# armando-palacio/opticomlib

Measured on AMD Instinct MI355X. Metric: SSFM sample*steps/sec, 2^20-sample dual-pol fiber, higher is better.
Workload: dtype c64

## Files before the change

opticomlib_amd/csrc/ssfm_host.hip:

```cpp
#include <hip/hip_runtime.h>

#include <algorithm>
#include <memory>
#include <cmath>
#include <cstdarg>
#include <cstddef>
#include <cstdio>
#include <cstdlib>
#include <chrono>
#include <cstring>
#include <atomic>
#include <condition_variable>
#include <functional>
#include <mutex>
#include <new>
#include <string>
#include <thread>
#include <type_traits>
#include <vector>

#include "ssfm_amd.h"
#include "ssfm_common.hpp"
#include "ssfm_kernels.hpp"
#include "ssfm_launch.hpp"
#include "ssfm_medium.hpp"
#include "ssfm_owned.hpp"
#include "ssfm_schedule.hpp"
#include "ssfm_split.hpp"

using namespace ssfm;

namespace {

constexpr int kLog2Min = 8, kLog2Max = 24;
constexpr int kLog2MaxDirect = 22;
template <typename T> constexpr int cols_per_tile() { return sizeof(T) == 8 ? 8 : 16; }
constexpr int kMaxTables = 4;

constexpr int freq_rows(int n2, int e) { return (n2 / e) >= 64 ? 1 : ((64 * e / n2) > 16 ? 16 : (64 * e / n2)); }

template <typename T, int MODE, int N1, int E>
hipError_t launch_time_n1(dim3 grid, hipStream_t s, const TimeArgs<T>& a) {
    constexpr int C = cols_per_tile<T>();
    constexpr bool U16 = u16_layout<T>(N1, C, E);
    if constexpr (!U16 && MODE > TM_END && MODE != TM_MID_A && MODE != TM_MID_L) return hipErrorInvalidValue;
    else if constexpr (U16 && MODE == TM_MID_L) return hipErrorInvalidValue;
    else if constexpr (MODE == TM_MID_A && N1 != 128 && N1 != 256) return hipErrorInvalidValue;
    else {
    constexpr size_t lds = col_pass_lds<T>(N1, C, E);
    if constexpr (MODE == TM_BEGIN || MODE == TM_MID || MODE == TM_END) {
        if (a.scal != nullptr)
            return launch_kernel<k_time<T, N1, C, E, MODE, U16, true>, lds>(grid, dim3(N1 * C / E), s, SSFM_TIME_KERNEL_ARGS(a));
    }
    return launch_kernel<k_time<T, N1, C, E, MODE, U16>, lds>(grid, dim3(N1 * C / E), s, SSFM_TIME_KERNEL_ARGS(a));
    }
}
template <typename T, int MODE, int E>
hipError_t launch_time_e(int N1, int batch, hipStream_t s, const TimeArgs<T>& a) {
    const dim3 grid((unsigned)(a.N2 / cols_per_tile<T>()) * batch);
    switch (N1) {
        case 16:  return launch_time_n1<T, MODE, 16, E>(grid, s, a);
        case 32:  return launch_time_n1<T, MODE, 32, E>(grid, s, a);
        case 64:  return launch_time_n1<T, MODE, 64, E>(grid, s, a);
        case 128: return launch_time_n1<T, MODE, 128, E>(grid, s, a);
        case 256: return launch_time_n1<T, MODE, 256, E>(grid, s, a);
        case 512: if constexpr (E == 16) return launch_time_n1<T, MODE, 512, E>(grid, s, a); else break;
    }
    return hipErrorInvalidValue;
}
template <typename T, int MODE>
hipError_t launch_time(int N1, int batch, hipStream_t s, TimeArgs<T> a, int E) {
    a.rows = batch;
    return E == 8 ? launch_time_e<T, MODE, 8>(N1, batch, s, a) : launch_time_e<T, MODE, 16>(N1, batch, s, a);
}

template <typename T, int MODE, int N2, int E, bool U16>
hipError_t launch_freq_u(int nrows, hipStream_t s, const FreqArgs<T>& a) {
    constexpr int ROWS = freq_rows(N2, E);
    constexpr size_t lds = row_pass_lds<T>(N2, E, ROWS);
    if constexpr (MODE == FM_FWD_ONLY || MODE == FM_INV_ONLY)
        return launch_kernel<k_freq_half<T, N2, ROWS, E, MODE, U16>, lds>(dim3(nrows / ROWS), dim3(ROWS * N2 / E), s, SSFM_FREQ_KERNEL_ARGS(a));
    else
        return launch_kernel<k_freq<T, N2, ROWS, E, MODE, U16>, lds>(dim3(nrows / ROWS), dim3(ROWS * N2 / E), s, SSFM_FREQ_KERNEL_ARGS(a));
}
template <typename T, int MODE, int N2, int E>
hipError_t launch_freq_n2(int nrows, hipStream_t s, const FreqArgs<T>& a) {
    if constexpr (sizeof(T) == 4)
        if (a.u16) return launch_freq_u<T, MODE, N2, E, true>(nrows, s, a);
    if constexpr ((MODE == FM_PHASE && sizeof(T) == 4) || MODE == FM_FLY_IM) return hipErrorInvalidValue;
    else return launch_freq_u<T, MODE, N2, E, false>(nrows, s, a);
}
template <typename T, int MODE, int E>
hipError_t launch_freq_e(int N2, int nrows, hipStream_t s, const FreqArgs<T>& a) {
    if constexpr (MODE == FM_INV_ONLY) {
        switch (N2) {
            case 4096: return launch_freq_n2<T, MODE, 4096, E>(nrows, s, a);
            case 8192: if constexpr (E == 16) return launch_freq_n2<T, MODE, 8192, E>(nrows, s, a); else break;
        }
        return hipErrorInvalidValue;
    } else
    switch (N2) {
        case 16:   return launch_freq_n2<T, MODE, 16, E>(nrows, s, a);
        case 32:   return launch_freq_n2<T, MODE, 32, E>(nrows, s, a);
        case 64:   return launch_freq_n2<T, MODE, 64, E>(nrows, s, a);
        case 128:  return launch_freq_n2<T, MODE, 128, E>(nrows, s, a);
        case 256:  return launch_freq_n2<T, MODE, 256, E>(nrows, s, a);
        case 512:  return launch_freq_n2<T, MODE, 512, E>(nrows, s, a);
        case 1024: return launch_freq_n2<T, MODE, 1024, E>(nrows, s, a);
        case 2048: return launch_freq_n2<T, MODE, 2048, E>(nrows, s, a);
        case 4096: return launch_freq_n2<T, MODE, 4096, E>(nrows, s, a);
        case 8192: if constexpr (E == 16) return launch_freq_n2<T, MODE, 8192, E>(nrows, s, a); else break;
    }
    return hipErrorInvalidValue;
}
template <typename T, int MODE>
hipError_t launch_freq(int N2, int nrows, hipStream_t s, FreqArgs<T> a, int E) {
    a.rows = nrows / a.N1;
    return E == 8 ? launch_freq_e<T, MODE, 8>(N2, nrows, s, a) : launch_freq_e<T, MODE, 16>(N2, nrows, s, a);
}

template <int MODE, int N1, int E>
hipError_t launch_time_h_n1(dim3 grid, hipStream_t s, const TimeArgs<double>& a) {
    constexpr int C = cols_per_tile<double>();
    return launch_kernel<k_time_h<double, N1, C, E, MODE>, col_pass_lds<double>(N1, C, E)>(grid, dim3(N1 * C / E), s, SSFM_TIME_KERNEL_ARGS(a));
}
constexpr bool line_half_shape(int N1, int N2, int E, int Ef) { return ((N1 == 256 && E == 8) || (N1 == 512 && E == 16)) && Ef == 16 && N2 >= 1024 && N2 <= 8192; }
template <int MODE>
hipError_t launch_time_h(int N1, int batch, hipStream_t s, TimeArgs<double> a, int E) {
    a.rows = batch;
    const dim3 grid((unsigned)(a.N2 / cols_per_tile<double>()) * batch);
    if (N1 == 256 && E == 8) return launch_time_h_n1<MODE, 256, 8>(grid, s, a);
    if (N1 == 512 && E == 16) return launch_time_h_n1<MODE, 512, 16>(grid, s, a);
    return hipErrorInvalidValue;
}
template <int N2>
hipError_t launch_freq_h_n2(int nrows, hipStream_t s, const FreqArgs<double>& a, const int* done) {
    constexpr int E = 16, ROWS = freq_rows(N2, E);
    constexpr auto kernel = &k_freq_h<double, N2, ROWS, E, FM_TABLE>;
    constexpr size_t lds = row_pass_lds<double>(N2, E, ROWS);
    const dim3 grid(nrows / ROWS), block(ROWS * N2 / E);
#if SSFM_TRACE
    return launch_kernel<kernel, lds>(grid, block, s, a.F, a.tab, a.tw2, a.st, a.h, a.amp, a.inv_n, a.step, a.N1, a.rows, a.u16, done, a.trace, a.trace_slot);
#else
    return launch_kernel<kernel, lds>(grid, block, s, a.F, a.tab, a.tw2, a.st, a.h, a.amp, a.inv_n, a.step, a.N1, a.rows, a.u16, done);
#endif
}
inline hipError_t launch_freq_h(int N2, int nrows, hipStream_t s, FreqArgs<double> a, const int* done = nullptr) {
    a.rows = nrows / a.N1;
    switch (N2) {
        case 1024: return launch_freq_h_n2<1024>(nrows, s, a, done);
        case 2048: return launch_freq_h_n2<2048>(nrows, s, a, done);
        case 4096: return launch_freq_h_n2<4096>(nrows, s, a, done);
        case 8192: return launch_freq_h_n2<8192>(nrows, s, a, done);
    }
    return hipErrorInvalidValue;
}

template <typename T, int MODE, int R>
hipError_t launch_split_mid_r(hipStream_t s, const SplitArgs<T>& a) {
    constexpr int V = split_positions<T, R>();
    const long long units = (long long)a.N1 * a.N2 / V;
    hipLaunchKernelGGL((k_split_mid<T, R, MODE>), dim3((unsigned)((units + 255) / 256)), dim3(256), 0, s, a);
    return hipGetLastError();
}
template <typename T, int MODE>
hipError_t launch_split_mid(int R, hipStream_t s, const SplitArgs<T>& a) {
    switch (R) {
        case 2:  return launch_split_mid_r<T, MODE, 2>(s, a);
        case 4:  return launch_split_mid_r<T, MODE, 4>(s, a);
        case 8:  return launch_split_mid_r<T, MODE, 8>(s, a);
        case 16: return launch_split_mid_r<T, MODE, 16>(s, a);
    }
    return hipErrorInvalidValue;
}
template <typename T, bool TO_SUB>
hipError_t launch_split_shuffle(int R, hipStream_t s, cx<T>* sub, cx<T>* nat, long long M, int rows) {
    const dim3 grid((unsigned)((M * rows + 255) / 256));
    switch (R) {
        case 2:  hipLaunchKernelGGL((k_split_shuffle<T, 2, TO_SUB>), grid, dim3(256), 0, s, sub, nat, M, rows); break;
        case 4:  hipLaunchKernelGGL((k_split_shuffle<T, 4, TO_SUB>), grid, dim3(256), 0, s, sub, nat, M, rows); break;
        case 8:  hipLaunchKernelGGL((k_split_shuffle<T, 8, TO_SUB>), grid, dim3(256), 0, s, sub, nat, M, rows); break;
        case 16: hipLaunchKernelGGL((k_split_shuffle<T, 16, TO_SUB>), grid, dim3(256), 0, s, sub, nat, M, rows); break;
        default: return hipErrorInvalidValue;
    }
    return hipGetLastError();
}

constexpr int kSmallE16Min = 4096;
template <typename T> constexpr int small_points(int n) { return sizeof(T) == 4 && n >= kSmallE16Min ? 16 : 8; }
template <typename T> constexpr bool small_supported(int n) {
    return n >= 256 && n <= (sizeof(T) == 4 ? 8192 : 4096) && (n & (n - 1)) == 0;
}
static_assert(kSmallTabs == kMaxTables, "k_small takes one table per cached step size");
template <int MAXN, typename F>
hipError_t small_size(int n, F&& f) {
    switch (n) {
        case 256:  return f(std::integral_constant<int, 256>());
        case 512:  return f(std::integral_constant<int, 512>());
        case 1024: return f(std::integral_constant<int, 1024>());
        case 2048: return f(std::integral_constant<int, 2048>());
        case 4096: return f(std::integral_constant<int, 4096>());
        case 8192: if constexpr (MAXN >= 8192) return f(std::integral_constant<int, 8192>()); else break;
    }
    return hipErrorInvalidValue;
}
template <typename T>
hipError_t launch_small(int n, int rows, hipStream_t s, const SmallArgs<T>& a) {
    return small_size<(sizeof(T) == 4 ? 8192 : 4096)>(n, [&](auto size) {
        constexpr int N = decltype(size)::value, E = small_points<T>(N);
        return launch_kernel<k_small<T, N, E>, row_pass_lds<T>(N, E, 1)>(dim3(rows), dim3(N / E), s, a);
    });
}

template <typename T> __device__ __forceinline__ cx<T> cm_chirp_value(long long m, long long n, int conj) {
    const long long r = (m * m) % (2 * n);
    double sn, cs;
    sincospi(-(double)r / (double)n, &sn, &cs);
    return mk<T>((T)cs, (T)(conj ? -sn : sn));
}
template <typename T> __global__ __launch_bounds__(256) void k_cm_kernel_line(cx<T>* __restrict__ F, long long n, long long M, int which) {
    for (long long i = (long long)blockIdx.x * blockDim.x + threadIdx.x; i < M; i += (long long)gridDim.x * blockDim.x) {
        const long long m = i < n ? i : (M - i < n ? M - i : -1);
        F[i] = m < 0 ? mk<T>((T)0, (T)0) : cm_chirp_value<T>(m, n, which == 0);
    }
}
template <typename T> __global__ __launch_bounds__(256) void k_cm_mul_table(const cx<T>* __restrict__ Dt, cx<T>* __restrict__ out, long long n, long long M, T h, T inv) {
    for (long long i = (long long)blockIdx.x * blockDim.x + threadIdx.x; i < M; i += (long long)gridDim.x * blockDim.x) {
        cx<T> d = mk<T>((T)0, (T)0);
        if (i < n) {
            const cx<T> x = Dt[i];
            const T xr = x.x * h, xi = x.y * h;
            const T e = (T)exp((double)xr);
            double sn, cs;
            sincos((double)xi, &sn, &cs);
            d = mk<T>((e * (T)cs) * inv, (e * (T)sn) * inv);
        }
        out[i] = d;
    }
}
__global__ __launch_bounds__(256) void k_cm_narrow(const cx<double>* __restrict__ src, cx<float>* __restrict__ dst, long long M, int conj) {
    for (long long i = (long long)blockIdx.x * blockDim.x + threadIdx.x; i < M; i += (long long)gridDim.x * blockDim.x)
        dst[i] = mk<float>((float)src[i].x, (float)(conj ? -src[i].y : src[i].y));
}
template <typename T> __global__ __launch_bounds__(256) void k_cm_pre(const cx<T>* __restrict__ A, const cx<T>* __restrict__ chirp, cx<T>* __restrict__ F, long long n, long long M, int batch) {
    const long long total = M * batch;
    for (long long i = (long long)blockIdx.x * blockDim.x + threadIdx.x; i < total; i += (long long)gridDim.x * blockDim.x) {
        const long long r = i / M, m = i - r * M;
        F[i] = m < n ? cmul(A[r * n + m], chirp[m]) : mk<T>((T)0, (T)0);
    }
}
template <typename T> __global__ __launch_bounds__(256) void k_cm_post(cx<T>* __restrict__ A, const cx<T>* __restrict__ chirp, const cx<T>* __restrict__ F, long long n, long long M, int batch,
                                                                      const unsigned* __restrict__ error) {
    if (*error != 0u) return;
    const long long total = n * batch;
    for (long long i = (long long)blockIdx.x * blockDim.x + threadIdx.x; i < total; i += (long long)gridDim.x * blockDim.x) {
        const long long r = i / n, m = i - r * n;
        A[i] = cmulc(F[r * M + m], chirp[m]);
    }
}

template <typename T> constexpr int chirp_points(int n) { return small_points<T>(n); }
template <typename T>
hipError_t launch_small_chirp(int n, int rows, hipStream_t s, const SmallChirpArgs<T>& a) {
    return small_size<4096>(n, [&](auto size) {
        constexpr int N = decltype(size)::value, E = chirp_points<T>(N);
        constexpr size_t lds = row_pass_lds<T>(N, E, 1, N);
        static_assert(lds <= 160 * 1024, "k_small_chirp: the line, its twiddles and H must fit the LDS");
        return launch_kernel<k_small_chirp<T, N, E>, lds>(dim3(rows), dim3(N / E), s, a);
    });
}
template <typename T>
hipError_t launch_small_chirp_adapt(int n, int rows, hipStream_t s, const SmallChirpAdaptArgs<T>& a) {
    return small_size<4096>(n, [&](auto size) {
        constexpr int N = decltype(size)::value, E = chirp_points<T>(N);
        constexpr size_t lds = row_pass_lds<T>(N, E, 1, N);
        static_assert(lds + 256 <= 160 * 1024, "k_small_chirp_adapt: the line, its twiddles and H must fit the LDS");
        return launch_kernel<k_small_chirp_adapt<T, N, E>, lds>(dim3(rows), dim3(N / E), s, a);
    });
}

template <typename T> constexpr bool small_adapt_supported(int n, int rows) {
    return small_supported<T>(n) && n <= 4096 && rows >= 1 && rows <= 2 && rows * n / small_points<T>(n) <= 512;
}
template <typename T, int N, int ROWS>
hipError_t launch_small_adapt_nr(hipStream_t s, const SmallAdaptArgs<T>& a) {
    constexpr int E = small_points<T>(N);
    if constexpr (ROWS * N / E <= 512) return launch_kernel<k_small_adapt<T, N, E, ROWS>, row_pass_lds<T>(N, E, ROWS)>(dim3(1), dim3(ROWS * N / E), s, a);
    else return hipErrorInvalidValue;
}
template <typename T>
hipError_t launch_small_adapt(int n, int rows, hipStream_t s, const SmallAdaptArgs<T>& a) {
    return small_size<4096>(n, [&](auto size) {
        constexpr int N = decltype(size)::value;
        return rows == 1 ? launch_small_adapt_nr<T, N, 1>(s, a) : launch_small_adapt_nr<T, N, 2>(s, a);
    });
}

class LaneWorker {
  public:
    ~LaneWorker() { stop(); }
    void start(int device) {
        if (th_.joinable()) return;
        th_ = std::thread([this, device] {
            (void)hipSetDevice(device);
            std::unique_lock<std::mutex> lk(m_);
            for (;;) {
                cv_.wait(lk, [this] { return has_job_ || quit_; });
                if (!has_job_) return;
                std::function<int()> job = std::move(job_);
                has_job_ = false;
                lk.unlock();
                const int rc = job();
                std::string err = rc != SSFM_OK ? std::string(ssfm::g_err) : std::string();
                lk.lock();
                rc_ = rc; err_ = std::move(err); done_ = true;
                cv_.notify_all();
            }
        });
    }
    void submit(std::function<int()> job) {
        std::lock_guard<std::mutex> lk(m_);
        job_ = std::move(job); has_job_ = true; done_ = false;
        cv_.notify_all();
    }
    int wait() {
        std::unique_lock<std::mutex> lk(m_);
        cv_.wait(lk, [this] { return done_; });
        if (rc_ != SSFM_OK) std::snprintf(ssfm::g_err, sizeof(ssfm::g_err), "%s", err_.c_str());
        return rc_;
    }
    void stop() {
        { std::lock_guard<std::mutex> lk(m_); quit_ = true; cv_.notify_all(); }
        if (th_.joinable()) th_.join();
    }
  private:
    std::thread th_;
    std::mutex m_;
    std::condition_variable cv_;
    std::function<int()> job_;
    bool has_job_ = false, done_ = false, quit_ = false;
    int rc_ = SSFM_OK;
    std::string err_;
};

__global__ void k_queue_probe_wait(unsigned* flag, unsigned* seen, long long patience) {
    const long long t0 = wall_clock64();
    unsigned v = 0u;
    while ((v = __hip_atomic_load(flag, __ATOMIC_RELAXED, __HIP_MEMORY_SCOPE_AGENT)) == 0u && wall_clock64() - t0 < patience) __builtin_amdgcn_s_sleep(8);
    *seen = v;
}
__global__ void k_queue_probe_set(unsigned* flag) { __hip_atomic_store(flag, 1u, __ATOMIC_RELAXED, __HIP_MEMORY_SCOPE_AGENT); }
__global__ void k_queue_probe_spin(long long ticks) {
    const long long t0 = wall_clock64();
    while (wall_clock64() - t0 < ticks) __builtin_amdgcn_s_sleep(4);
}
int streams_run_side_by_side(hipStream_t a, hipStream_t b, unsigned* words , hipEvent_t ev) {
    unsigned seen = 0u;
    if (hipMemsetAsync(words, 0, 2 * sizeof(unsigned), a) != hipSuccess) return -1;
    if (hipEventRecord(ev, a) != hipSuccess || hipStreamWaitEvent(b, ev, 0) != hipSuccess) return -1;
    hipLaunchKernelGGL(k_queue_probe_wait, dim3(1), dim3(1), 0, a, words, words + 1, 20000ll);
    hipLaunchKernelGGL(k_queue_probe_set, dim3(1), dim3(1), 0, b, words);
    if (hipGetLastError() != hipSuccess) return -1;
    if (hipMemcpyAsync(&seen, words + 1, sizeof(unsigned), hipMemcpyDeviceToHost, a) != hipSuccess) return -1;
    if (hipStreamSynchronize(a) != hipSuccess || hipStreamSynchronize(b) != hipSuccess) return -1;
    return seen != 0u ? 1 : 0;
}

constexpr float kLaneGoodRatio = 1.6f;
constexpr float kLaneGoodRatioBig = 2.1f;
constexpr float kLaneSlowRatio = 1.8f;
constexpr float kLaneSuspectRatio = 1.3f;
constexpr int kLaneDroppedCooldown = 32;
constexpr int kLaneProbeSteps = 12;
constexpr int kLaneHealsMax = 8;

struct LanePair { int device; hipStream_t main, lane; float score, alone_us, pair_us; };
struct LanePool {
    std::mutex m;
    std::vector<LanePair> free;
    static constexpr size_t kMax = 8;
    bool take(int device, LanePair* out) {
        std::lock_guard<std::mutex> lk(m);
        for (size_t i = free.size(); i-- > 0;)
            if (free[i].device == device) { *out = free[i]; free.erase(free.begin() + (long)i); return true; }
        return false;
    }
    bool give(const LanePair& p) {
        std::lock_guard<std::mutex> lk(m);
        if (free.size() >= kMax) return false;
        free.push_back(p);
        return true;
    }
};
LanePool& lane_pool() { static LanePool* p = new LanePool(); return *p; }
std::atomic<long long> g_lane_ratings{0}, g_lane_pairs_reused{0};

struct PlanBase {
    int precision = 0;
    virtual ~PlanBase() {}
};

constexpr int kMaxLanesConst = 8;
template <typename T> struct PlanT : PlanBase {
    int device = 0;
    int64_t n = 0;
    int batch = 0;
    int N1 = 0, N2 = 0;
    hipStream_t stream = nullptr;
    Event ev0, ev1;
    cx<T>* F = nullptr;
    cx<T>* Y = nullptr;
    T* P = nullptr;
    DeviceBuffer<cx<T>> F_own, Y_own;
    DeviceBuffer<T> P_own;
    DeviceBuffer<cx<T>> twN;
    DeviceBuffer<cx<T>> twA;
    DeviceBuffer<cx<T>> twB;
    DeviceBuffer<cx<T>> tw1;
    DeviceBuffer<cx<T>> tw2;
    DeviceBuffer<cx<T>> dnat;
    DeviceBuffer<cx<T>> dperm;
    DeviceBuffer<cx<T>> dperm_fly;
    DeviceBuffer<T> dimag_fly;
    bool dimag_valid = false;
    DeviceBuffer<cx<T>> tw2_fly;
    DeviceBuffer<cx<T>> scratch;
    DeviceBuffer<cx<T>> xfer_tab[2];
    struct Tab { T h = 0; DeviceBuffer<cx<T>> ptr; bool valid = false; int kind = 0; };
    Tab tabs[kMaxTables];
    bool op_flat_re = false;
    T op_re0 = 0;
    bool phase_tables = true;
    bool force_fly = false;
    int tab_rr = 0;
    bool small = false;
    DeviceBuffer<cx<T>> tw_small;
    DeviceBuffer<cx<T>> tw_chirp;
    DeviceBuffer<cx<T>> dsmall;
    bool medium_ok = true;
    static constexpr size_t kSet = kBarShards + kBarWords + 2;
    DeviceBuffer<unsigned long long> medium_st;
    PinnedBuffer<unsigned> medium_err_host;
    Stream medium_stream2;
    Event medium_ev2;
    bool medium_pending = false;
    bool medium_split_ok = true;
    bool medium_adapt_ok = true;
    static constexpr long long medium_max_samples = 1ll << 17;
    int medium_xcc = -1, medium_xccs = 8;
    std::vector<T> medium_sched;
    double medium_gamma = 0;
    long long medium_patience = 2000000ll;
    bool fused_ok = true;
    DeviceBuffer<cx<T>> fused_backup;
    Tab stabs[kMaxTables];
    int stab_rr = 0;
    DeviceBuffer<T> d_hs;
    std::vector<unsigned char> h_sched;
    DeviceBuffer<AdaptState<T>> st;
    DeviceBuffer<T> zlog;
    bool have_op = false;
    int split_R = 1;
    int64_t n_full = 0;
    int batch_full = 0;
// ... 2368 lines not shown
```

opticomlib_amd/csrc/ssfm_split.hpp:

```cpp
#pragma once
#include "ssfm_kernels.hpp"

namespace ssfm {

constexpr int kSplitLog2M = 20;
constexpr int kSplitMaxR = 16;

enum SplitMode { SM_TABLE = 0, SM_FLY = 1, SM_PHASE = 2 };

template <typename T> struct SplitArgs {
    cx<T>* Y;
    const cx<T>* G;
    const double2* twA;
    const double2* twB;
    const AdaptState<T>* st;
    T h;
    T inv_n;
    T amp;
    int step;
    int N1, N2;
    int rows_outer;
    int Qf;
};
__host__ __device__ __forceinline__ long long split_k2_of_pos(long long pos, int Qf) { return Qf > 0 ? u16_col_of_pos(pos, Qf) : pos; }

template <typename T, int R> __host__ __device__ constexpr int split_positions() { return sizeof(T) == 4 ? 2 : 1; }
template <typename T, int R, int MODE>
__global__ __launch_bounds__(256) void k_split_mid(const SplitArgs<T> a) {
    constexpr int V = split_positions<T, R>();
    typedef T v4_t __attribute__((ext_vector_type(V * 2)));
    const long long M = (long long)a.N1 * a.N2;
    const long long unit = (long long)blockIdx.x * 256 + threadIdx.x;
    if (unit * V >= M) return;
    const long long p0 = unit * V;
    const int k1 = (int)(p0 / a.N2);
    int k2v[V];
#pragma unroll
    for (int v = 0; v < V; ++v) k2v[v] = (int)split_k2_of_pos(p0 % a.N2 + v, a.Qf);
    T h = a.h;
    if (MODE == SM_FLY && a.st != nullptr) {
        const StepState<T> S = a.st->cur[a.step & 1];
        if (S.done || a.st->error != 0u) return;
        h = S.h;
    }
    cx<T> g[R][V];
    if constexpr (MODE == SM_PHASE) {
        typedef unsigned uv_t __attribute__((ext_vector_type(V)));
        const unsigned* Gu = reinterpret_cast<const unsigned*>(a.G);
#pragma unroll
        for (int p = 0; p < R; ++p) {
            const uv_t q = *reinterpret_cast<const uv_t*>(Gu + (long long)p * M + p0);
#pragma unroll
            for (int v = 0; v < V; ++v) g[p][v] = phase32_factor(q[v], a.amp);
        }
    } else {
#pragma unroll
    for (int p = 0; p < R; ++p) {
        const v4_t q = *reinterpret_cast<const v4_t*>(a.G + (long long)p * M + p0);
#pragma unroll
        for (int v = 0; v < V; ++v) g[p][v] = mk<T>(q[2 * v], q[2 * v + 1]);
    }
    }
    if constexpr (MODE == SM_FLY) {
#pragma unroll
        for (int v = 0; v < V; ++v) {
            cx<T> m[R];
            T ph[R];
            bool flat = true;
#pragma unroll
            for (int p = 0; p < R; ++p) { m[p] = g[p][v]; ph[p] = m[p].y * h; flat = flat && (m[p].x == m[0].x); }
            const T e0 = exp_acc<T>(m[0].x * h);
            fly_factors<R>(m, ph, flat, e0, h, a.inv_n);
#pragma unroll
            for (int p = 0; p < R; ++p) g[p][v] = m[p];
        }
    }
    cx<T> w[R][V];
#pragma unroll
    for (int s = 1; s < R; ++s) {
        const double2 A = a.twA[s * a.N1 + k1];
#pragma unroll
        for (int v = 0; v < V; ++v) {
            const double2 B = a.twB[(long long)s * a.N2 + k2v[v]];
            w[s][v] = mk<T>((T)(A.x * B.x - A.y * B.y), (T)(A.x * B.y + A.y * B.x));
        }
    }
    for (int row = 0; row < a.rows_outer; ++row) {
        cx<T>* base = a.Y + (long long)row * R * M + p0;
        cx<T> y[R][V];
#pragma unroll
        for (int s = 0; s < R; ++s) {
            const v4_t q = *reinterpret_cast<const v4_t*>(base + (long long)s * M);
#pragma unroll
            for (int v = 0; v < V; ++v) y[s][v] = mk<T>(q[2 * v], q[2 * v + 1]);
        }
#pragma unroll
        for (int v = 0; v < V; ++v) {
            cx<T> t[R];
            t[0] = y[0][v];
#pragma unroll
            for (int s = 1; s < R; ++s) t[s] = cmul(y[s][v], w[s][v]);
            Dft<R>::template run<-1>(t);
#pragma unroll
            for (int p = 0; p < R; ++p) t[p] = cmul(t[p], g[p][v]);
            Dft<R>::template run<+1>(t);
            y[0][v] = t[0];
#pragma unroll
            for (int s = 1; s < R; ++s) y[s][v] = cmul(t[s], mk<T>(w[s][v].x, -w[s][v].y));
        }
#pragma unroll
        for (int s = 0; s < R; ++s) {
            v4_t q;
#pragma unroll
            for (int v = 0; v < V; ++v) { q[2 * v] = y[s][v].x; q[2 * v + 1] = y[s][v].y; }
            *reinterpret_cast<v4_t*>(base + (long long)s * M) = q;
        }
    }
}

template <typename T, int MODE>
__global__ void k_make_split_table(const cx<T>* __restrict__ src, cx<T>* __restrict__ out, int N1, int N2, int R, T h, T inv_n, int Qf) {
    const long long o = (long long)blockIdx.x * blockDim.x + threadIdx.x;
    const long long M = (long long)N1 * N2;
    if (o >= M * R) return;
    const long long p = o / M, r = o % M;
    const long long k1 = r / N2, k2 = split_k2_of_pos(r % N2, Qf);
    cx<T> d = src[k1 + (long long)N1 * k2 + M * p];
    if (MODE == 1) { d.x *= inv_n; d.y *= inv_n; }
    if (MODE == 2) {
        const T xr = d.x * h, xi = d.y * h;
        const T e = (T)exp((double)xr);
        double s, c;
        sincos((double)xi, &s, &c);
        d.x = (e * (T)c) * inv_n;
        d.y = (e * (T)s) * inv_n;
    }
    out[o] = d;
}
template <typename T>
__global__ void k_make_split_phase_table(const cx<T>* __restrict__ src, unsigned* __restrict__ out, int N1, int N2, int R, T h, int Qf) {
    const long long o = (long long)blockIdx.x * blockDim.x + threadIdx.x;
    const long long M = (long long)N1 * N2;
    if (o >= M * R) return;
    const long long p = o / M, r = o % M;
    const long long k1 = r / N2, k2 = split_k2_of_pos(r % N2, Qf);
    const T xi = src[k1 + (long long)N1 * k2 + M * p].y * h;
    double turns = (double)xi * 0.15915494309189533577;
    turns -= floor(turns);
    out[o] = (unsigned)(unsigned long long)llrint(turns * 4294967296.0);
}
template <typename T>
__global__ void k_make_split_dm_table(cx<T>* __restrict__ out, cx<T>* __restrict__ nat, int N1, int N2, int R, double val, double D, T inv_n, int Qf) {
    const long long o = (long long)blockIdx.x * blockDim.x + threadIdx.x;
    const long long M = (long long)N1 * N2, N = M * R;
    if (o >= N) return;
    const long long p = o / M, r = o % M;
    const long long k = (r / N2) + (long long)N1 * split_k2_of_pos(r % N2, Qf) + M * p;
    const long long ks = k < (N + 1) / 2 ? k : k - N;
    const double w = ((double)ks * val) * 2.0 * 3.141592653589793;
    const double ph = ((w * w) * D) / 2.0;
    double s, c;
    sincos(ph, &s, &c);
    out[o] = mk<T>((T)c * inv_n, (T)s * inv_n);
    if (nat != nullptr) nat[k] = mk<T>((T)c, (T)s);
}
__global__ inline void k_make_split_twiddles(double2* twA, double2* twB, int N1, int N2, int R) {
    const long long o = (long long)blockIdx.x * blockDim.x + threadIdx.x;
    const long long N = (long long)N1 * N2 * R;
    const long long nA = (long long)R * N1, nB = (long long)R * N2;
    if (o >= nA + nB) return;
    long long m;
    if (o < nA) { const long long s = o / N1, k1 = o % N1; m = (s * k1) % N; }
    else { const long long s = (o - nA) / N2, k2 = (o - nA) % N2; m = ((s * N1) % N) * k2 % N; }
    double sn, cs;
    sincospi(-2.0 * (double)m / (double)N, &sn, &cs);
    (o < nA ? twA[o] : twB[o - nA]) = make_double2(cs, sn);
}
template <typename T, int R, bool TO_SUB>
__global__ __launch_bounds__(256) void k_split_shuffle(cx<T>* __restrict__ sub, cx<T>* __restrict__ nat, long long M, int rows) {
    const long long o = (long long)blockIdx.x * 256 + threadIdx.x;
    if (o >= M * rows) return;
    const long long row = o / M, m = o % M;
    cx<T>* n0 = nat + (row * M + m) * R;
    cx<T>* s0 = sub + row * R * M + m;
#pragma unroll
    for (int a = 0; a < R; ++a) {
        if (TO_SUB) s0[(long long)a * M] = n0[a];
        else n0[a] = s0[(long long)a * M];
    }
}

}
```

Measured before the change: 67.41 billion.

## Split radix-16 mid kernel across four waves with LDS exchange

Adds a specialized fp32 radix-16 split-mid kernel in which each of four wavefronts handles four of the sixteen sub-signals. The 16-point DFT becomes two radix-4 stages with an LDS transpose between them, and each block covers 128 positions. This is meant to cut per-thread register pressure and raise occupancy compared with one thread holding all 16 points. It also adds compile-time ablation switches to the generic kernel that skip twiddles or phases, for experiments. The cost is two __syncthreads and LDS traffic per row, and the path is used only when N2 is divisible by 128.

```diff
diff --git a/opticomlib_amd/csrc/ssfm_host.hip b/opticomlib_amd/csrc/ssfm_host.hip
--- a/opticomlib_amd/csrc/ssfm_host.hip
+++ b/opticomlib_amd/csrc/ssfm_host.hip
@@ -160,6 +160,12 @@
 hipError_t launch_split_mid_r(hipStream_t s, const SplitArgs<T>& a) {
     constexpr int V = split_positions<T, R>();
     const long long units = (long long)a.N1 * a.N2 / V;
+    if constexpr (R == 16 && sizeof(T) == 4 && MODE != SM_FLY && SSFM_SPLIT16_ABLATE == 0) {
+        if (a.N2 % kSplit16Pos == 0) {
+            hipLaunchKernelGGL((k_split_mid16<MODE>), dim3((unsigned)((long long)a.N1 * a.N2 / kSplit16Pos)), dim3(kSplit16Block), 0, s, a);
+            return hipGetLastError();
+        }
+    }
     hipLaunchKernelGGL((k_split_mid<T, R, MODE>), dim3((unsigned)((units + 255) / 256)), dim3(256), 0, s, a);
     return hipGetLastError();
 }
diff --git a/opticomlib_amd/csrc/ssfm_split.hpp b/opticomlib_amd/csrc/ssfm_split.hpp
--- a/opticomlib_amd/csrc/ssfm_split.hpp
+++ b/opticomlib_amd/csrc/ssfm_split.hpp
@@ -25,9 +25,14 @@
 __host__ __device__ __forceinline__ long long split_k2_of_pos(long long pos, int Qf) { return Qf > 0 ? u16_col_of_pos(pos, Qf) : pos; }
 
 template <typename T, int R> __host__ __device__ constexpr int split_positions() { return sizeof(T) == 4 ? 2 : 1; }
+#ifndef SSFM_SPLIT16_ABLATE
+#define SSFM_SPLIT16_ABLATE 0
+#endif
 template <typename T, int R, int MODE>
 __global__ __launch_bounds__(256) void k_split_mid(const SplitArgs<T> a) {
     constexpr int V = split_positions<T, R>();
+    constexpr int ABL = (R == 16 && MODE == SM_PHASE && sizeof(T) == 4) ? SSFM_SPLIT16_ABLATE : 0;
+    constexpr bool kNoTw = ABL == 1 || ABL == 2 || ABL == 3, kNoPh = ABL == 1 || ABL == 2 || ABL == 4;
     typedef T v4_t __attribute__((ext_vector_type(V * 2)));
     const long long M = (long long)a.N1 * a.N2;
     const long long unit = (long long)blockIdx.x * 256 + threadIdx.x;
@@ -44,7 +49,12 @@
         h = S.h;
     }
     cx<T> g[R][V];
-    if constexpr (MODE == SM_PHASE) {
+    if constexpr (kNoPh) {
+#pragma unroll
+        for (int p = 0; p < R; ++p)
+#pragma unroll
+            for (int v = 0; v < V; ++v) g[p][v] = mk<T>(a.amp, a.inv_n);
+    } else if constexpr (MODE == SM_PHASE) {
         typedef unsigned uv_t __attribute__((ext_vector_type(V)));
         const unsigned* Gu = reinterpret_cast<const unsigned*>(a.G);
 #pragma unroll
@@ -76,6 +86,7 @@
         }
     }
     cx<T> w[R][V];
+    if constexpr (!kNoTw)
 #pragma unroll
     for (int s = 1; s < R; ++s) {
         const double2 A = a.twA[s * a.N1 + k1];
@@ -94,19 +105,25 @@
 #pragma unroll
             for (int v = 0; v < V; ++v) y[s][v] = mk<T>(q[2 * v], q[2 * v + 1]);
         }
+        if constexpr (ABL == 1) {
+#pragma unroll
+            for (int s = 0; s < R; s += 2)
+#pragma unroll
+                for (int v = 0; v < V; ++v) { const cx<T> t = y[s][v]; y[s][v] = y[s + 1][v]; y[s + 1][v] = t; }
+        } else
 #pragma unroll
         for (int v = 0; v < V; ++v) {
             cx<T> t[R];
             t[0] = y[0][v];
 #pragma unroll
-            for (int s = 1; s < R; ++s) t[s] = cmul(y[s][v], w[s][v]);
+            for (int s = 1; s < R; ++s) t[s] = kNoTw ? y[s][v] : cmul(y[s][v], w[s][v]);
             Dft<R>::template run<-1>(t);
 #pragma unroll
             for (int p = 0; p < R; ++p) t[p] = cmul(t[p], g[p][v]);
             Dft<R>::template run<+1>(t);
             y[0][v] = t[0];
 #pragma unroll
-            for (int s = 1; s < R; ++s) y[s][v] = cmul(t[s], mk<T>(w[s][v].x, -w[s][v].y));
+            for (int s = 1; s < R; ++s) y[s][v] = kNoTw ? t[s] : cmul(t[s], mk<T>(w[s][v].x, -w[s][v].y));
         }
 #pragma unroll
         for (int s = 0; s < R; ++s) {
@@ -115,6 +132,141 @@
             for (int v = 0; v < V; ++v) { q[2 * v] = y[s][v].x; q[2 * v + 1] = y[s][v].y; }
             *reinterpret_cast<v4_t*>(base + (long long)s * M) = q;
         }
+    }
+}
+
+constexpr int kSplit16Block = 256;
+constexpr int kSplit16Pos = 128;
+template <int DIR, int B> __device__ __forceinline__ void split16_twiddle(cf32* x) {
+    using K = RadixConst<float>;
+    if constexpr (B == 1) {
+        x[1] = cmuld<DIR>(x[1], mk<float>(K::cA, -K::sA));
+        x[2] = add_rot<DIR>(x[2], x[2]);
+        x[3] = cmuld<DIR>(x[3], mk<float>(K::sB, -K::cB));
+    } else if constexpr (B == 2) {
+        x[1] = add_rot<DIR>(x[1], x[1]);
+        x[2] = rot90<DIR>(x[2]);
+        x[3] = sub_rot<DIR>(x[3], x[3]);
+    } else if constexpr (B == 3) {
+        x[1] = cmuld<DIR>(x[1], mk<float>(K::sB, -K::cB));
+        x[2] = sub_rot<DIR>(x[2], x[2]);
+        x[3] = cmuld<DIR>(x[3], mk<float>(-K::cB, K::sB));
+    }
+}
+template <int Q> __device__ __forceinline__ void split16_scale(cf32* x) {
+    using K = RadixConst<float>;
+    if constexpr (Q == 1) x[2] = scale2(x[2], mk<float>(K::R2D, K::R2D));
+    if constexpr (Q == 2) { x[1] = scale2(x[1], mk<float>(K::R2D, K::R2U)); x[3] = scale2(x[3], mk<float>(-K::R2D, -K::R2D)); }
+    if constexpr (Q == 3) x[2] = scale2(x[2], mk<float>(-K::R2D, -K::R2U));
+}
+template <int B> __device__ __forceinline__ void split16_exchange(float4* lds, int lane, cf32 (&x)[4][2]) {
+#pragma unroll
+    for (int q = 0; q < 4; ++q) lds[(B * 4 + q) * 64 + lane] = make_float4(x[q][0].x, x[q][0].y, x[q][1].x, x[q][1].y);
+    __syncthreads();
+#pragma unroll
+    for (int b = 0; b < 4; ++b) {
+        const float4 t = lds[(b * 4 + B) * 64 + lane];
+        x[b][0] = mk<float>(t.x, t.y);
+        x[b][1] = mk<float>(t.z, t.w);
+    }
+}
+template <int B, int MODE>
+__device__ __forceinline__ void split16_body(const SplitArgs<float>& a, float4* lds, int lane) {
+    typedef float v4_t __attribute__((ext_vector_type(4)));
+    const long long M = (long long)a.N1 * a.N2;
+    const long long p0 = ((long long)blockIdx.x * (kSplit16Pos / 2) + lane) * 2;
+    const int k1 = (int)((long long)blockIdx.x * kSplit16Pos / a.N2);
+    int k2v[2];
+#pragma unroll
+    for (int v = 0; v < 2; ++v) k2v[v] = (int)split_k2_of_pos(p0 % a.N2 + v, a.Qf);
+    cf32 g[4][2];
+#pragma unroll
+    for (int j = 0; j < 4; ++j) {
+        const long long o = (long long)(B + 4 * j) * M + p0;
+        if constexpr (MODE == SM_PHASE) {
+            const uint2 q = *reinterpret_cast<const uint2*>(reinterpret_cast<const unsigned*>(a.G) + o);
+            g[j][0] = phase32_factor(q.x, a.amp);
+            g[j][1] = phase32_factor(q.y, a.amp);
+        } else {
+            const v4_t q = *reinterpret_cast<const v4_t*>(a.G + o);
+            g[j][0] = mk<float>(q[0], q[1]);
+            g[j][1] = mk<float>(q[2], q[3]);
+        }
+    }
+    cf32 w[4][2];
+#pragma unroll
+    for (int j = 0; j < 4; ++j) {
+        const int s = B + 4 * j;
+        if (s == 0) continue;
+        const double2 A = a.twA[s * a.N1 + k1];
+#pragma unroll
+        for (int v = 0; v < 2; ++v) {
+            const double2 Bv = a.twB[(long long)s * a.N2 + k2v[v]];
+            w[j][v] = mk<float>((float)(A.x * Bv.x - A.y * Bv.y), (float)(A.x * Bv.y + A.y * Bv.x));
+        }
+    }
+    for (int row = 0; row < a.rows_outer; ++row) {
+        cf32* base = a.Y + (long long)row * 16 * M + p0;
+        cf32 x[4][2];
+#pragma unroll
+        for (int j = 0; j < 4; ++j) {
+            const v4_t q = *reinterpret_cast<const v4_t*>(base + (long long)(B + 4 * j) * M);
+            x[j][0] = mk<float>(q[0], q[1]);
+            x[j][1] = mk<float>(q[2], q[3]);
+        }
+#pragma unroll
+        for (int v = 0; v < 2; ++v) {
+            cf32 t[4];
+#pragma unroll
+            for (int j = 0; j < 4; ++j) t[j] = (B + 4 * j == 0) ? x[j][v] : cmul(x[j][v], w[j][v]);
+            dft4<-1>(t[0], t[1], t[2], t[3]);
+            split16_twiddle<-1, B>(t);
+#pragma unroll
+            for (int j = 0; j < 4; ++j) x[j][v] = t[j];
+        }
+        split16_exchange<B>(lds, lane, x);
+#pragma unroll
+        for (int v = 0; v < 2; ++v) {
+            cf32 t[4];
+#pragma unroll
+            for (int j = 0; j < 4; ++j) t[j] = x[j][v];
+            split16_scale<B>(t);
+            dft4<-1>(t[0], t[1], t[2], t[3]);
+#pragma unroll
+            for (int j = 0; j < 4; ++j) t[j] = cmul(t[j], g[j][v]);
+            dft4<+1>(t[0], t[1], t[2], t[3]);
+            split16_twiddle<+1, B>(t);
+#pragma unroll
+            for (int j = 0; j < 4; ++j) x[j][v] = t[j];
+        }
+        split16_exchange<B>(lds + 16 * 64, lane, x);
+#pragma unroll
+        for (int v = 0; v < 2; ++v) {
+            cf32 t[4];
+#pragma unroll
+            for (int j = 0; j < 4; ++j) t[j] = x[j][v];
+            split16_scale<B>(t);
+            dft4<+1>(t[0], t[1], t[2], t[3]);
+#pragma unroll
+            for (int j = 0; j < 4; ++j) x[j][v] = (B + 4 * j == 0) ? t[j] : cmul(t[j], mk<float>(w[j][v].x, -w[j][v].y));
+        }
+#pragma unroll
+        for (int j = 0; j < 4; ++j) {
+            v4_t q;
+            q[0] = x[j][0].x; q[1] = x[j][0].y; q[2] = x[j][1].x; q[3] = x[j][1].y;
+            *reinterpret_cast<v4_t*>(base + (long long)(B + 4 * j) * M) = q;
+        }
+    }
+}
+template <int MODE>
+__global__ __launch_bounds__(kSplit16Block) void k_split_mid16(const SplitArgs<float> a) {
+    __shared__ float4 lds[2 * 16 * 64];
+    const int lane = threadIdx.x & 63;
+    switch (__builtin_amdgcn_readfirstlane(threadIdx.x >> 6)) {
+        case 0: split16_body<0, MODE>(a, lds, lane); break;
+        case 1: split16_body<1, MODE>(a, lds, lane); break;
+        case 2: split16_body<2, MODE>(a, lds, lane); break;
+        default: split16_body<3, MODE>(a, lds, lane); break;
     }
 }
 
```

Result: slower. 66.57 billion (-1.2%).
